# coralogix/arrow-ballista

Hardware: AMD Instinct MI355X
Metric: tpch_sf100_q3_lineitem_rows_per_sec (higher is better)
Workload: dtype i128; 1 GPU; TPC-H SF100 q3 (BASELINE configs[2]): filter x3 + hash join customer|x|orders + hash join |x| lineitem + aggregate + sort, one task on 1 x MI355X; lineitem_rows=600037902, lineitem_rows_per_gpu=600037902, orders_rows_per_gpu=150009476, customer_rows_per_gpu=15000000, input=Arrow-physical columns resident in HBM, parallelism=single partition

## Files before the change

### arrow-ballista_amd/csrc/capi.cpp

```cpp
#include "../../include/gpuq.h"
#include "expr_compile.h"
#include "agg_compile.h"
#include "gpuq_kernels.h"
#include "jit_runtime.h"
#include "devbuf.h"
#include "gpuq_internal.h"
#include <hip/hip_runtime.h>
#include <algorithm>
#include <memory>
#include <mutex>
#include <cctype>
#include <cstdio>
#include <cstdlib>
#include <cstring>
#include <string>
#include <tuple>
#include <map>
#include <deque>
#include <functional>
#include <vector>

using namespace gpuq;

namespace {
// ... 15 lines not shown
  Schema in_schema;
  CompiledProgram prog;
  DevBuf code_dev, flags_dev;
  std::vector<gpuq_field_info> out_fields;
  std::string mode = "Single", strategy = "auto";
  AggSpec agg{}; KeySpec keys{};
  std::vector<DType> key_types, acc_types;
  std::vector<int> acc_bits;
  std::map<std::pair<const void*, int>, int> jit_runs;
  std::map<std::tuple<const void*, int, size_t>, const JitFn*> jit_fns;
  struct PostChunk { CompiledProgram prog; DevBuf code; int first_out = 0; };
  std::deque<PostChunk> posts; Schema post_schema;
  i64 expected_groups = 0;
  int join_type = JT_INNER; int null_eq = 0; bool build_side_rows = true;
  bool has_semi = false; KeySpec semi_keys{};
  SortSpec sort{}; i64 fetch = -1;
  uint32_t nparts = 0;
  struct { void* data = nullptr; u64* valid = nullptr; bool done = false; } sort_dec;
  DType sort_key0;
  std::string refuse;
  std::string label;
  bool deferred = false, defer_client = false;
  struct Learned {
    struct { bool valid = false, dense = false, sparse_bits = false, has_dups = false; i64 kmin = 0; u64 krange = 0; } jb;
    struct { bool valid = false; int path = 0, gmax = 0; u64 est = 0; bool use_lds = false; i64 groups = -1; } ag;
    struct { bool valid = false; SortPack K{}; int total = 0; } so;
    bool join_guess_failed = false, sort_guess_failed = false;
    uint32_t expect_flags = 0;
    void forget() { jb.valid = ag.valid = so.valid = false; }
  } learned;
  DevBuf ws[10];
  uint32_t* pin = nullptr;
  uint32_t* pinned() { if (!pin) { if (hipHostMalloc((void**)&pin, 256, hipHostMallocDefault) != hipSuccess) { (void)hipGetLastError(); pin = nullptr; } } return pin; }
  bool profile = false; hipEvent_t ev0 = nullptr, ev1 = nullptr; float kernel_ms = 0; int launches = 0; bool ev_pending = false;
  hipEvent_t ev2 = nullptr, ev3 = nullptr; float total_ms = 0, last_total_ms = 0; bool ev_total_pending = false;
  ~gpuq_op() { for (hipEvent_t e : {ev0, ev1, ev2, ev3}) if (e) (void)hipEventDestroy(e); if (pin) (void)hipHostFree(pin); }
};

struct gpuq_join_table {
  gpuq_ctx* ctx = nullptr;
  KeySpec keys{}; HashTable T{}; int null_eq = 0; bool has_present = true;
  DevBuf slots, dense, dense_bits, next, visited, present, ws_bitmap, ws_counts;
  i64 bound = 0;
  bool visited_ready = false;
  bool has_dups = false;
};

// ... 48 lines not shown
  return P;
}

void need_exact_rows(const gpuq_input* in, const char* what) {
  if (in && in->n_rows_dev) throw std::runtime_error(std::string(what) + ": the input carries a device-side row count (n_rows_dev); this entry point needs the exact count");
}
void reset_flags(gpuq_op* op, hipStream_t s) { HIPCHECK(hipMemsetAsync(op->flags_dev.p, 0, 4, s)); }
void read_status(gpuq_op* op, hipStream_t s, uint32_t* out, int n) {
  uint32_t* h = op->pinned();
  HIPCHECK(hipMemcpyAsync(h ? h : out, op->flags_dev.p, (size_t)n * 4, hipMemcpyDeviceToHost, s));
  HIPCHECK(hipStreamSynchronize(s));
  if (h) for (int i = 0; i < n; ++i) out[i] = h[i];
}
uint32_t read_flags(gpuq_op* op, hipStream_t s) { uint32_t f = 0; read_status(op, s, &f, 1); return f; }
void raise_flags(uint32_t f) {
  if (f & FLAG_STR_TRUNC) throw Unsupported("a Utf8 value longer than 15 bytes reached a device string comparison/key (PACKED15 limit)");
  if (f & FLAG_DEC_OVERFLOW) throw std::runtime_error("decimal arithmetic overflow: a result or a rescaled operand does not fit Decimal128 (38 digits / 127 bits)");
  if (f & FLAG_WIDE_MINMAX) throw Unsupported("MIN/MAX over a value outside the int64 range is not supported on device");
  if (f & FLAG_DUP_BUILD_KEY) throw Unsupported("duplicate build keys without a chain buffer");
  if (f & FLAG_OUT_OVERFLOW) throw Capacity("join output capacity exceeded; see the pair count for the required size");
  if (f & FLAG_TABLE_FULL) throw std::runtime_error("hash table full");
  if (f & FLAG_GROUP_OVERFLOW) throw Capacity("group capacity exceeded");
  if (f & FLAG_SORT_LAYOUT) throw std::runtime_error("a row does not fit the remembered sort key layout");
}

struct ProfScope {
  gpuq_op* op; hipStream_t s;
  ProfScope(gpuq_op* o, hipStream_t st) : op(o), s(st) {
    if (op->profile) {
      if (!op->ev0) { HIPCHECK(hipEventCreate(&op->ev0)); HIPCHECK(hipEventCreate(&op->ev1)); }
      if (op->ev_pending) { float ms = 0; HIPCHECK(hipEventSynchronize(op->ev1)); HIPCHECK(hipEventElapsedTime(&ms, op->ev0, op->ev1)); op->kernel_ms += ms; op->ev_pending = false; }
      HIPCHECK(hipEventRecord(op->ev0, s));
    }
  }
  ~ProfScope() { if (op->profile) { (void)hipEventRecord(op->ev1, s); op->ev_pending = true; op->launches++; } }
};

struct ProfTotal {
  gpuq_op* op; hipStream_t s; bool on = false;
  ProfTotal(gpuq_op* o, hipStream_t st) : op(o), s(st) {
    if (op->profile) {
      if (!op->ev2) { HIPCHECK(hipEventCreate(&op->ev2)); HIPCHECK(hipEventCreate(&op->ev3)); }
      if (op->ev_total_pending) {
        if (hipEventQuery(op->ev3) != hipSuccess) { (void)hipGetLastError(); return; }
        float ms = 0; HIPCHECK(hipEventElapsedTime(&ms, op->ev2, op->ev3)); op->total_ms += ms; op->ev_total_pending = false;
      }
// ... 739 lines not shown
          cnt = std::min<u64>(cnt * (u64)wstep, (u64)n);
        }
        const u64 lim = std::max<u64>((u64)cnt * (u64)dense_ratio, 1ull << 16);
        if (span < (1ull << 31) && span < lim && (span + 1) * 4 <= op->ctx->hbm / 8) { dense = true; kmin = lo; krange = span + 1; sparse_bits = cnt * 4 < krange; }
      }
    }
    t->T.dense = nullptr; t->T.dense_bits = nullptr; t->T.dense_min = 0; t->T.dense_range = 0;
    if (dense) {
      t->T.n_slots = 0; t->T.slots = nullptr;
      t->T.dense = (uint32_t*)t->dense.ensure((size_t)krange * 4 + 16); t->T.dense_min = kmin; t->T.dense_range = krange;
      if (sparse_bits) {
        const size_t bb = ((size_t)krange + 63) / 64 * 8 + 8;
        t->T.dense_bits = (uint32_t*)t->dense_bits.ensure(bb);
        HIPCHECK(hipMemsetAsync(t->T.dense_bits, 0, bb, s));
      } else HIPCHECK(hipMemsetAsync(t->T.dense, 0xFF, (size_t)krange * 4, s));
    } else {
      t->T.n_slots = next_pow2(std::max<u64>((u64)n * 3, 1024));
      t->T.slots = (u64*)t->slots.ensure((size_t)t->T.n_slots * t->T.slot_words * 8);
    }
    uint32_t* next = (!memo || jb.has_dups) ? (uint32_t*)t->next.ensure((size_t)std::max<i64>(build_rows_bound, 1) * 4) : nullptr;
    const size_t bm = ((size_t)build_rows_bound + 63) / 64 * 8 + 8;
    uint32_t* present = op->build_side_rows ? (uint32_t*)t->present.ensure(bm) : nullptr;
    t->has_present = op->build_side_rows;
    auto build = [&]() {
      if (present) HIPCHECK(hipMemsetAsync(present, 0, bm, s));
      if (!dense) launch_ht_init(s, t->T, nullptr);
      if (!memo) reset_flags(op, s);
      if (rows_out) HIPCHECK(hipMemsetAsync(rows_out, 0, 8, s));
      { SinkJit jit(op, op->prog, GPUQ_SINK_JOIN_BUILD, n, semi_spec(t->T, present)); ProfScope ps(op, s); if (!launch_join_build(s, jit.fn, P, n, op->keys, t->T, next, present, payload_via, op->null_eq, semi_p)) throw Unsupported("join build over a semi table: more than 8 input columns without the specialised kernel"); }
      HIPCHECK(hipGetLastError());
    };
    build();
    if (memo) { t->has_dups = jb.has_dups; return true; }
    uint32_t f = read_flags(op, s);
    if (guess && (f & FLAG_TABLE_FULL)) { reset_flags(op, s); return false; }
    if (sparse_bits && (f & FLAG_DUP_BUILD_KEY)) {
      t->T.dense_bits = nullptr;
      HIPCHECK(hipMemsetAsync(t->T.dense, 0xFF, (size_t)krange * 4, s));
      build();
      f = read_flags(op, s);
    }
    if (f & ~FLAG_DUP_BUILD_KEY) { reset_flags(op, s); raise_flags(f & ~FLAG_DUP_BUILD_KEY); }
    if (f) reset_flags(op, s);
    t->has_dups = (f & FLAG_DUP_BUILD_KEY) != 0;
    jb = {true, dense, t->T.dense_bits != nullptr, t->has_dups, kmin, krange};
    op->learned.expect_flags = t->has_dups ? FLAG_DUP_BUILD_KEY : 0u;
    return true;
    };
    bool built = false;
    static const bool trace = getenv("GPUQ_TRACE_JOIN_BUILD") != nullptr;
    if (op->deferred && op->learned.jb.valid) { built = attempt(2); if (trace) fprintf(stderr, "[gpuq] join build: %lld rows (bound), deferred with the remembered layout\n", (long long)n); }
    else if (in->n_rows_dev) throw std::runtime_error("join build: a device-side row count needs a deferred operator with a completed synchronous run (gpuq_op_can_defer)");
    if (!built && spec_on && narrow_key && n >= (1ll << 21) && !op->learned.join_guess_failed) { built = attempt(true); if (!built) op->learned.join_guess_failed = true; if (trace) fprintf(stderr, "[gpuq] join build: %lld rows, guessed range %s\n", (long long)n, built ? "held" : "did not hold"); }
    if (!built) { attempt(false); if (trace) fprintf(stderr, "[gpuq] join build: %lld rows, measured range, %s\n", (long long)n, t->T.dense ? (t->T.dense_bits ? "array + bitmap" : "array") : "hash table"); }
    *out = t;
  });
  if (rc != GPUQ_OK) { delete t; if (out) *out = nullptr; }
  return rc;
}
int gpuq_join_build_run(gpuq_op* op, void* stream, const gpuq_input* in, int payload_via, int64_t build_rows_bound, gpuq_join_table** out) {
  return join_build_impl(op, stream, in, payload_via, build_rows_bound, nullptr, nullptr, nullptr, out);
}
int gpuq_join_build_run_semi(gpuq_op* op, void* stream, const gpuq_input* in, int payload_via, int64_t build_rows_bound, gpuq_join_table* semi_table,
                             uint32_t* semi_hits_out, uint64_t* rows_out, gpuq_join_table** out) {
  if (!semi_table) return GPUQ_ERR_INVALID;
  return join_build_impl(op, stream, in, payload_via, build_rows_bound, semi_table, semi_hits_out, rows_out, out);
}
int gpuq_join_table_has_duplicates(const gpuq_join_table* t) { return t && t->has_dups ? 1 : 0; }
// ... 900 lines not shown
```

### arrow-ballista_amd/csrc/gpuq_dev.h

```cpp
#pragma once
#ifndef __HIPCC_RTC__
#include <hip/hip_runtime.h>
#include <stdint.h>
#else
typedef signed char int8_t;
typedef unsigned char uint8_t;
typedef signed short int16_t;
typedef unsigned short uint16_t;
typedef signed int int32_t;
typedef unsigned int uint32_t;
#endif

namespace gpuq {

typedef unsigned long long u64;
typedef long long i64;
typedef __int128 i128;
typedef unsigned __int128 u128;

constexpr int MAX_COLS = 16;
constexpr int NREG = 16;
constexpr int MAX_INSNS = 192;
constexpr int MAX_IMMS = 48;
constexpr int MAX_VIA = 3;
// ... 59 lines not shown
  const uint32_t* via[MAX_VIA];
  const DevCode* code;
  uint32_t* flags;
  const u64* n_dev;
};
#ifdef GPUQ_NT_STREAM
#define GPUQ_LD_STREAM(p) __builtin_nontemporal_load(p)
#else
#define GPUQ_LD_STREAM(p) (*(p))
#endif
__device__ __forceinline__ i64 rows_of(const DevProgram& P, const i64 n_bound) {
  if (P.n_dev) { const i64 nd = (i64)*P.n_dev; return nd < n_bound ? nd : n_bound; }
  return n_bound;
}

constexpr uint32_t FLAG_STR_TRUNC = 1u;
constexpr uint32_t FLAG_GROUP_OVERFLOW = 2u;
constexpr uint32_t FLAG_TABLE_FULL = 4u;
constexpr uint32_t FLAG_DUP_BUILD_KEY = 8u;
constexpr uint32_t FLAG_OUT_OVERFLOW = 16u;
constexpr uint32_t FLAG_WIDE_MINMAX = 32u;
constexpr uint32_t FLAG_DEC_OVERFLOW = 128u;
constexpr uint32_t FLAG_SORT_LAYOUT = 64u;

#define GPUQ_REGS_DECL ::gpuq::u64 rlo[::gpuq::NREG]; ::gpuq::u64 rhi[::gpuq::NREG]; uint32_t rnulls = 0
#define GPUQ_REGS_PARAM ::gpuq::u64 (&rlo)[::gpuq::NREG], ::gpuq::u64 (&rhi)[::gpuq::NREG], uint32_t& rnulls
#define GPUQ_REGS_CPARAM const ::gpuq::u64 (&rlo)[::gpuq::NREG], const ::gpuq::u64 (&rhi)[::gpuq::NREG], const uint32_t& rnulls
#define GPUQ_REGS rlo, rhi, rnulls

__device__ __forceinline__ i128 mk128(u64 lo, u64 hi) { return (i128)(((u128)hi << 64) | (u128)lo); }

__device__ __forceinline__ i64 f64_total_key(u64 bits) {
  i64 s = (i64)bits;
  return s ^ (i64)((u64)(s >> 63) >> 1);
}

__device__ __forceinline__ void str15_assemble(u64 w0, u64 w1, u64 w2, uint32_t byte_off, int32_t n, u64& hi, u64& lo) {
  hi = 0; lo = 0;
  if (n <= 0) return;
  const uint32_t sh = byte_off * 8u;
  u64 s0 = sh ? ((w0 >> sh) | (w1 << (64u - sh))) : w0;
  u64 s1 = sh ? ((w1 >> sh) | (w2 << (64u - sh))) : w1;
  if (n < 8) { s0 &= (1ull << (8 * n)) - 1; s1 = 0; }
  else if (n == 8) s1 = 0;
  else s1 &= (1ull << (8 * (n - 8))) - 1;
  hi = __builtin_bswap64(s0); lo = __builtin_bswap64(s1);
// ... 323 lines not shown
```

### arrow-ballista_amd/csrc/gpuq_kernels.h

```cpp
#pragma once
#include "gpuq_dev.h"
#ifndef GPUQ_JIT
#include <type_traits>
#include "devbuf.h"
#endif

namespace gpuq {

constexpr int MAX_OUTS = 16;
struct OutCol {
  void* data;
  u64* validity;
  int32_t reg;
  int32_t cls;
};
struct OutSpec { int32_t n_out; int32_t pad; OutCol cols[MAX_OUTS]; };

constexpr int MAX_ACCS = 12;
constexpr int MAX_KEYS = 4;
enum AccKind : int32_t { ACC_SUM = 0, ACC_COUNT = 1, ACC_COUNT_STAR = 2, ACC_MIN = 3, ACC_MAX = 4, ACC_FSUM = 5, ACC_FMIN = 6, ACC_FMAX = 7 };
struct AggSpec {
  int32_t n_keys, n_accs;
  int32_t key_reg[MAX_KEYS];
  int32_t acc_kind[MAX_ACCS];
// ... 6 lines not shown



constexpr int MAX_KW = 2 * MAX_KEYS + 1;
struct KeySpec {
  int32_t n_keys;
  int32_t key_reg[MAX_KEYS];
  int32_t key_wide[MAX_KEYS];
  int32_t null_word;
  int32_t key_words;
  int32_t word_reg[MAX_KW];
  int32_t word_half[MAX_KW];
};
struct HashTable {
  u64* slots;
  u64 n_slots;
  int32_t slot_words;
  int32_t key_words;
  uint32_t* dense;
  i64 dense_min;
  u64 dense_range;
  uint32_t* dense_bits;
};
struct SemiProbe { HashTable T; KeySpec K; int32_t null_eq; int32_t on; uint32_t* hit_out; u64* rows_out; };
enum JoinType : int32_t { JT_INNER = 0, JT_LEFT = 1, JT_RIGHT = 2, JT_FULL = 3, JT_LEFT_SEMI = 4, JT_LEFT_ANTI = 5, JT_RIGHT_SEMI = 6, JT_RIGHT_ANTI = 7 };


constexpr uint32_t NIL = 0xFFFFFFFFu;
__device__ __forceinline__ uint32_t tag_of(u64 h) { return (uint32_t)(h >> 32) | 2u; }

__device__ __forceinline__ u64 acc_identity(const int kind, const int half) {
  switch (kind) {
    case ACC_MIN: return half ? 0 : 0x7FFFFFFFFFFFFFFFull;
    case ACC_MAX: return half ? ~0ull : 0x8000000000000000ull;
    case ACC_FMIN: return half ? 0 : 0x7FF0000000000000ull;
    case ACC_FMAX: return half ? 0 : 0xFFF0000000000000ull;
    default: return 0;
  }
}
__device__ __forceinline__ u64 slot_word_identity(const AggSpec& A, const int w, const int cell0) {
  const int a = (w - cell0) >> 1;
  return (w >= cell0 && a < A.n_accs) ? acc_identity(A.acc_kind[a], (w - cell0) & 1) : 0;
}
__device__ __forceinline__ void lds_table_init(u64* slots, const uint32_t cap, const int slot_words, const int cell0, const AggSpec& A, const uint32_t nthreads) {
  for (uint32_t i = threadIdx.x; i < cap * (uint32_t)slot_words; i += nthreads) slots[i] = slot_word_identity(A, (int)(i % (uint32_t)slot_words), cell0);
}
__device__ __forceinline__ bool acc_operand(const AggSpec& A, const int a, GPUQ_REGS_CPARAM, u64& vlo, u64& vhi) {
// ... 174 lines not shown
int agg_tiny_max_groups(int n_accs);
size_t agg_tiny_workspace_bytes(int gmax, int n_keys, int n_accs, int* nblocks_out);
void launch_agg_tiny(hipStream_t s, void* jit_fn, const DevProgram& P, i64 n, const AggSpec& A, int gmax, void* workspace);
void launch_agg_tiny_merge(hipStream_t s, const DevProgram& P, i64 n, const AggSpec& A, int gmax, void* workspace, const AggOut& out);
void launch_ht_init(hipStream_t s, const HashTable& T, const AggSpec* A);
void launch_agg_hash(hipStream_t s, void* jit_fn, const DevProgram& P, i64 n, const KeySpec& K, const AggSpec& A, const HashTable& T);
void launch_key_sample(hipStream_t s, const DevProgram& P, i64 n, const KeySpec& K, i64 stride, i64 nsample, uint32_t* bitmap, u64 nbits, unsigned long long* passed);
uint32_t agg_lds_slots(const HashTable& T);
int agg_lds_grid(i64 n);
void launch_agg_lds(hipStream_t s, void* jit_fn, const DevProgram& P, i64 n, const KeySpec& K, const AggSpec& A, const HashTable& T, u64* fstage, int n_fsum);
void launch_agg_bucket_id(hipStream_t s, void* jit_fn, const DevProgram& P, i64 n, const KeySpec& K, u64 bucket_mask, u64* bid, uint32_t* ids);
void launch_bucket_bounds(hipStream_t s, const u64* sorted_bid, i64 n, u64 nbuckets, uint32_t* bounds, int shift);
void launch_agg_bucket(hipStream_t s, void* jit_fn, const DevProgram& P, const KeySpec& K, const AggSpec& A, const uint32_t* ids, const uint32_t* bounds, uint32_t nbuckets,
                       uint32_t cap, int slot_words, const AggOut& out);
void launch_agg_hash_extract(hipStream_t s, const KeySpec& K, const AggSpec& A, const HashTable& T, const AggOut& out, uint32_t* flags);
bool launch_join_build(hipStream_t s, void* jit_fn, const DevProgram& P, i64 n, const KeySpec& K, const HashTable& T, uint32_t* next, uint32_t* present,
                       int payload_via, int null_equals_null, const SemiProbe* semi = nullptr);
void launch_join_keyrange(hipStream_t s, void* jit_fn, const DevProgram& P, i64 n, const KeySpec& K, int null_equals_null, u64* out, i64 wstep = 1);
void launch_join_probe_unique(hipStream_t s, void* jit_fn, const DevProgram& P, i64 n, const KeySpec& K, const HashTable& T, int join_type, int null_equals_null, int payload_via,
                              uint32_t* seg_build, uint32_t* seg_probe, uint32_t* seg_counts, int nsegs, i64 wpw, uint32_t* visited);
void launch_copy_segments(hipStream_t s, const uint32_t* seg_build, const uint32_t* seg_probe, const uint32_t* seg_offsets, int nsegs, i64 wpw, i64 n,
                          const u64* total, uint32_t* out_build, uint32_t* out_probe, u64 out_cap, uint32_t* flags);
void launch_join_locality(hipStream_t s, const DevProgram& P, i64 n, const KeySpec& K, const HashTable& T, i64 stride, i64 nsample, u64* out);
struct RjGeomHost { uint32_t nparts, shift; i64 tile; int32_t nblocks; };
void rj_geometry(i64 n, u64 range, int slice_log2, RjGeomHost* g);
size_t rj_hist_entries(const RjGeomHost& g);
void launch_rj_partition(hipStream_t s, void* jit_fn, const DevProgram& P, i64 n, const KeySpec& K, const HashTable& T, int payload_via, const RjGeomHost& g,
                         u64* rec, u64* rec_out, int32_t* hist, void* scan_ws, size_t scan_ws_bytes);
int rj_probe_geometry(i64 n, i64* wpw_out);
void launch_rj_probe(hipStream_t s, const u64* rec, const int32_t* n_live, const HashTable& T, int join_type, uint32_t* seg_build, uint32_t* seg_probe,
                     uint32_t* seg_counts, int nblocks, i64 wpw);
void launch_bitmap_select(hipStream_t s, const u64* present, const u64* visited, int matched, i64 nwords, i64 n, u64* bitmap,
                          uint32_t* block_counts, int nblocks, i64 wpb);
void launch_join_probe(hipStream_t s, void* jit_fn, const DevProgram& P, i64 n, const KeySpec& K, const HashTable& T, const uint32_t* next,
                       int join_type, int payload_via, int null_equals_null, uint32_t* out_build, uint32_t* out_probe,
                       u64 out_cap, u64* out_count, uint32_t* visited);
int sort_minmax_blocks(i64 n);
void launch_sort_minmax(hipStream_t s, void* jit_fn, const DevProgram& P, i64 n, const SortSpec& S, u64* out, int nblocks, i64 wstep = 1);
int sort_max_passes();
void launch_sort_pack(hipStream_t s, void* jit_fn, const DevProgram& P, i64 n, const SortSpec& S, const SortPack& K, u64* key_lo, u64* key_hi, uint32_t* ids, u64* hist, int hist_passes);
void launch_part_pid(hipStream_t s, void* jit_fn, const DevProgram& P, i64 n, const KeySpec& K, uint32_t nparts, u64* pid_out, uint32_t* ids);
void launch_part_offsets(hipStream_t s, const u64* pid, i64 n, uint32_t nparts, uint32_t* counts_ws, u64* offsets_out, int shift);
void launch_counts_to_ghist(hipStream_t s, const uint32_t* counts, uint32_t np, u64* ghist);
void launch_gather_u64(hipStream_t s, const u64* src, const uint32_t* idx, i64 n, u64* dst);
int sort_small_max();
int sort_direct_max();
// ... 110 lines not shown
```

### arrow-ballista_amd/csrc/kernels_hash.hip

```cpp
#include "gpuq_kernels.h"

namespace gpuq {

constexpr int HBLOCK = 256;
constexpr int HWAVES = HBLOCK / 64;

__device__ __forceinline__ int hlane() { return threadIdx.x & 63; }
__device__ __forceinline__ int hwave() { return threadIdx.x >> 6; }

__device__ __forceinline__ u64 a_load(const u64* p) { return __hip_atomic_load(p, __ATOMIC_RELAXED, __HIP_MEMORY_SCOPE_AGENT); }
__device__ __forceinline__ void a_store(u64* p, u64 v) { __hip_atomic_store(p, v, __ATOMIC_RELAXED, __HIP_MEMORY_SCOPE_AGENT); }
__device__ __forceinline__ u64 a_cas(u64* p, u64 expected, u64 desired) {
  __hip_atomic_compare_exchange_strong(p, &expected, desired, __ATOMIC_RELAXED, __ATOMIC_RELAXED, __HIP_MEMORY_SCOPE_AGENT);
  return expected;
}
__device__ __forceinline__ u64 a_add(u64* p, u64 v) { return __hip_atomic_fetch_add(p, v, __ATOMIC_RELAXED, __HIP_MEMORY_SCOPE_AGENT); }

__device__ __forceinline__ bool make_key(const KeySpec& K, GPUQ_REGS_CPARAM, u64 (&kw)[MAX_KW], u64& hash) {
  uint32_t knull = 0;
  u64 h = 0x243F6A8885A308D3ull;
#pragma unroll
  for (int k = 0; k < MAX_KEYS; ++k) {
    if (k < K.n_keys) {
      const int r = __builtin_amdgcn_readfirstlane(K.key_reg[k]);
// ... 514 lines not shown
  uint32_t payload;
  return ht_find(T, kw, h, payload) ? payload : NIL;
}

__device__ __forceinline__ void build_insert_dense(const DevProgram& P, const HashTable& T, uint32_t* __restrict__ next, const u64 idx, const uint32_t row) {
  bool inserted; uint32_t old = NIL;
  if (T.dense_bits) {
    const uint32_t bit = 1u << (idx & 31);
    const uint32_t was = atomicOr(T.dense_bits + (idx >> 5), bit);
    T.dense[idx] = row;
    inserted = !(was & bit);
  } else {
    old = __hip_atomic_exchange(T.dense + idx, row, __ATOMIC_RELAXED, __HIP_MEMORY_SCOPE_AGENT);
    inserted = old == NIL;
  }
  if (inserted) {
    if (next) next[row] = NIL;
  } else {
    if (!(__hip_atomic_load(P.flags, __ATOMIC_RELAXED, __HIP_MEMORY_SCOPE_AGENT) & FLAG_DUP_BUILD_KEY)) atomicOr(P.flags, FLAG_DUP_BUILD_KEY);
    if (next) next[row] = old;
  }
}
constexpr int BUILD_QCAP = 128;
template <int MAXC, bool SEMI>
__device__ __forceinline__ void k_join_build_body(const DevProgram P, const i64 n_arg, const KeySpec K, const HashTable T,
                                                       uint32_t* __restrict__ next, uint32_t* __restrict__ present, const int payload_via,
                                                       const int null_eq, const SemiProbe S) {
  const i64 n = rows_of(P, n_arg);
  __shared__ uint32_t q_pos[SEMI ? HWAVES : 1][SEMI ? BUILD_QCAP : 1], q_idx[SEMI ? HWAVES : 1][SEMI ? BUILD_QCAP : 1], q_aux[SEMI ? HWAVES : 1][SEMI ? BUILD_QCAP : 1];
  const bool queued = SEMI && S.on && T.dense != nullptr;
  const bool s_bits = S.T.dense != nullptr && S.T.dense_bits != nullptr;
  uint32_t qn = 0, survivors = 0;
  const int wv = SEMI ? hwave() : 0;
  auto flush = [&](const uint32_t from, const uint32_t cnt) {
    const bool on = (uint32_t)hlane() < cnt;
    const uint32_t j = from + (on ? (uint32_t)hlane() : 0u);
    const uint32_t pos = q_pos[wv][j], idx = q_idx[wv][j], aux = q_aux[wv][j];
    if (on) {
      if (S.hit_out) S.hit_out[pos] = s_bits ? S.T.dense[aux] : aux;
      build_insert_dense(P, T, next, (u64)idx, pos);
    }
  };
  for_rows_in_flight<MAXC>(P, n, (i64)blockIdx.x * HWAVES + hwave(), (i64)gridDim.x * HWAVES, [&](const i64 w, const i64 pos, bool active, GPUQ_REGS_PARAM) {
    uint32_t aux = NIL;
    if (SEMI && S.on) {
      bool found = false;
      if (active) {
        u64 kw1[MAX_KW]; u64 h1;
#pragma unroll
        for (int q = 0; q < MAX_KW; ++q) kw1[q] = 0;
        const bool null1 = make_key(S.K, GPUQ_REGS, kw1, h1);
        if (!(null1 && !S.null_eq)) {
          if (s_bits && queued) {
            const u64 i1 = kw1[0] - (u64)S.T.dense_min;
            if (i1 < S.T.dense_range && ((S.T.dense_bits[i1 >> 5] >> (i1 & 31)) & 1u)) { found = true; aux = (uint32_t)i1; }
          } else { aux = join_lookup(S.T, kw1, h1); found = aux != NIL; }
        }
      }
      active = active && found;
      if (!queued && active && S.hit_out) S.hit_out[pos] = aux;
      if (S.rows_out) survivors += active ? 1u : 0u;
    }
    if (present && payload_via == 0) { const u64 am = __ballot(active); if (hlane() == 0) ((u64*)present)[w] = am; }
    if (queued) {
      u64 idx = 0; bool ins = false;
      if (active) {
        u64 kw[MAX_KW]; u64 h;
#pragma unroll
        for (int q = 0; q < MAX_KW; ++q) kw[q] = 0;
        const bool any_null = make_key(K, GPUQ_REGS, kw, h);
        idx = kw[0] - (u64)T.dense_min;
        ins = !(any_null && !null_eq);
        if (ins && idx >= T.dense_range) { atomicOr(P.flags, FLAG_TABLE_FULL); ins = false; }
        if (!ins && S.hit_out) S.hit_out[pos] = s_bits ? S.T.dense[aux] : aux;
      }
      const u64 m = __ballot(ins);
      if (ins) {
        const uint32_t j = qn + (uint32_t)__popcll(m & ((1ull << hlane()) - 1));
        q_pos[wv][j] = (uint32_t)pos; q_idx[wv][j] = (uint32_t)idx; q_aux[wv][j] = aux;
      }
      qn += (uint32_t)__popcll(m);
      __builtin_amdgcn_fence(__ATOMIC_RELEASE, "wavefront"); __builtin_amdgcn_wave_barrier(); __builtin_amdgcn_fence(__ATOMIC_ACQUIRE, "wavefront");
      if (qn >= 64) { qn -= 64; flush(qn, 64); __builtin_amdgcn_wave_barrier(); }
      return;
    }
    if (!active) return;
    u64 kw[MAX_KW]; u64 h;
#pragma unroll
    for (int q = 0; q < MAX_KW; ++q) kw[q] = 0;
    const bool any_null = make_key(K, GPUQ_REGS, kw, h);
    uint32_t row = (uint32_t)pos;
    if (payload_via > 0) { row = P.via[payload_via - 1][pos]; if (present) atomicOr(&present[row >> 5], 1u << (row & 31)); }
    if (any_null && !null_eq) return;
    if (T.dense) {
      const u64 idx = kw[0] - (u64)T.dense_min;
      if (idx >= T.dense_range) { atomicOr(P.flags, FLAG_TABLE_FULL); return; }
      build_insert_dense(P, T, next, idx, row);
      return;
    }
    bool inserted; uint32_t old = NIL;
    const u64 s = ht_find_or_insert(T, kw, h, row, inserted);
    if (s == ~0ull) { atomicOr(P.flags, FLAG_TABLE_FULL); return; }
    if (!inserted && next) {
      uint32_t* head = (uint32_t*)(T.slots + s * (u64)T.slot_words) + 1;
      old = __hip_atomic_exchange(head, row, __ATOMIC_RELAXED, __HIP_MEMORY_SCOPE_AGENT);
    }
    if (inserted) {
      if (next) next[row] = NIL;
    } else {
      if (!(__hip_atomic_load(P.flags, __ATOMIC_RELAXED, __HIP_MEMORY_SCOPE_AGENT) & FLAG_DUP_BUILD_KEY)) atomicOr(P.flags, FLAG_DUP_BUILD_KEY);
      if (next) next[row] = old;
    }
  });
  if (queued && qn > 0) flush(0, qn);
  if (SEMI && S.on && S.rows_out) {
#pragma unroll
    for (int o = 32; o > 0; o >>= 1) survivors += __shfl_xor(survivors, o);
    if (hlane() == 0 && survivors) atomicAdd((unsigned long long*)S.rows_out, (unsigned long long)survivors);
  }
}
#if defined(GPUQ_JIT) && defined(GPUQ_JIT_SEMI) && GPUQ_JIT_SEMI == 2
template <int MAXC>
__device__ __forceinline__ void k_join_build_semi1_body(const DevProgram P, const i64 n_arg, const HashTable T, uint32_t* __restrict__ next, const SemiProbe S) {
#ifndef GPUQ_SEMI_ROWS
#define GPUQ_SEMI_ROWS 4
#endif
  constexpr int U = GPUQ_SEMI_ROWS;
  constexpr int QC = 64 * (U + 1);
  __shared__ uint32_t q_pos[HWAVES][QC], q_idx[HWAVES][QC], q_aux[HWAVES][QC];
  const i64 n = rows_of(P, n_arg);
  const i64 nwords = (n + 63) >> 6;
  const int wv = hwave();
  const bool s_dense = S.T.dense != nullptr;
  const uint32_t* __restrict__ sbits = S.T.dense_bits;
  const bool late_row = s_dense && sbits != nullptr;
  uint32_t qn = 0, survivors = 0;
  auto flush = [&](const uint32_t from, const uint32_t cnt) {
    const bool on = (uint32_t)hlane() < cnt;
    const uint32_t j = from + (on ? (uint32_t)hlane() : 0u);
    const uint32_t pos = q_pos[wv][j], idx = q_idx[wv][j], aux = q_aux[wv][j];
    if (on) {
      if (S.hit_out) S.hit_out[pos] = late_row ? S.T.dense[aux] : aux;
      build_insert_dense(P, T, next, (u64)idx, pos);
    }
  };
  const i64 wave0 = ((i64)blockIdx.x * HWAVES + hwave()) * U, wstride = (i64)gridDim.x * HWAVES * U;
  for (i64 wb = wave0; wb < nwords; wb += wstride) {
    bool act[U]; u64 key1[U], key2[U]; bool n1[U], n2[U]; i64 posc[U];
    {
      JitPre jq[U]; JitRaw jw[U];
#pragma unroll
      for (int u = 0; u < U; ++u) {
        const i64 pos = ((wb + u) << 6) + hlane();
        act[u] = (wb + u) < nwords && pos < n;
        posc[u] = act[u] ? pos : n - 1;
        gpuq_jit_pre(P, posc[u], jq[u]);
      }
#pragma unroll
      for (int u = 0; u < U; ++u) gpuq_jit_load(P, posc[u], jq[u], jw[u]);
#pragma unroll
      for (int u = 0; u < U; ++u) {
        GPUQ_REGS_DECL;
        const bool pass = gpuq_jit_compute(P, posc[u], jw[u], GPUQ_REGS);
        act[u] = act[u] && pass;
        n1[u] = (rnulls >> JIT_KEY_REG0) & 1; n2[u] = (rnulls >> JIT_KEY2_REG) & 1;
        key1[u] = rlo[JIT_KEY_REG0]; key2[u] = rlo[JIT_KEY2_REG];
      }
    }
    uint32_t aux[U]; bool found[U];
    if (s_dense) {
      uint32_t bw[U]; u64 i1[U]; bool in[U];
#pragma unroll
      for (int u = 0; u < U; ++u) {
        i1[u] = key1[u] - (u64)S.T.dense_min;
        in[u] = act[u] && !n1[u] && i1[u] < S.T.dense_range;
        bw[u] = 0;
        if (in[u]) bw[u] = sbits ? sbits[i1[u] >> 5] : S.T.dense[i1[u]];
      }
#pragma unroll
      for (int u = 0; u < U; ++u) {
        if (sbits) { found[u] = in[u] && ((bw[u] >> (i1[u] & 31)) & 1u); aux[u] = (uint32_t)i1[u]; }
        else { found[u] = in[u] && bw[u] != NIL; aux[u] = bw[u]; }
      }
    } else {
#pragma unroll
      for (int u = 0; u < U; ++u) {
        aux[u] = NIL;
        if (act[u] && !n1[u]) { u64 kw1[MAX_KW]; for (int q = 0; q < MAX_KW; ++q) kw1[q] = 0; kw1[0] = key1[u]; aux[u] = join_lookup(S.T, kw1, hash_combine(0x243F6A8885A308D3ull, key1[u], 0, false)); }
        found[u] = aux[u] != NIL;
      }
    }
#pragma unroll
    for (int u = 0; u < U; ++u) {
      const bool surv = act[u] && found[u];
      survivors += surv ? 1u : 0u;
      const u64 idx = key2[u] - (u64)T.dense_min;
      bool ins = surv && !n2[u];
      if (ins && idx >= T.dense_range) { atomicOr(P.flags, FLAG_TABLE_FULL); ins = false; }
      if (surv && !ins && S.hit_out) S.hit_out[posc[u]] = late_row ? S.T.dense[aux[u]] : aux[u];
      const u64 m = __ballot(ins);
      if (ins) {
        const uint32_t j = qn + (uint32_t)__popcll(m & ((1ull << hlane()) - 1));
        q_pos[wv][j] = (uint32_t)posc[u]; q_idx[wv][j] = (uint32_t)idx; q_aux[wv][j] = aux[u];
      }
      qn += (uint32_t)__popcll(m);
    }
    __builtin_amdgcn_fence(__ATOMIC_RELEASE, "wavefront"); __builtin_amdgcn_wave_barrier(); __builtin_amdgcn_fence(__ATOMIC_ACQUIRE, "wavefront");
    while (qn >= 64) { qn -= 64; flush(qn, 64); }
    __builtin_amdgcn_wave_barrier();
  }
  if (qn > 0) flush(0, qn);
  if (S.rows_out) {
#pragma unroll
    for (int o = 32; o > 0; o >>= 1) survivors += __shfl_xor(survivors, o);
    if (hlane() == 0 && survivors) atomicAdd((unsigned long long*)S.rows_out, (unsigned long long)survivors);
  }
}
#endif
#ifndef GPUQ_JIT
template <int MAXC, bool SEMI>
__global__ void __launch_bounds__(HBLOCK) k_join_build(const DevProgram P, const i64 n, const KeySpec K, const HashTable T,
                                                       uint32_t* __restrict__ next, uint32_t* __restrict__ present, const int payload_via,
                                                       const int null_eq, const SemiProbe S) { k_join_build_body<MAXC, SEMI>(P, n, K, T, next, present, payload_via, null_eq, S); }
#elif GPUQ_JIT_KERNEL == GPUQ_SINK_JOIN_BUILD
#ifndef GPUQ_JIT_SEMI
#define GPUQ_JIT_SEMI 0
#endif
extern "C" __global__ void __launch_bounds__(HBLOCK) gpuq_jit_entry(const DevProgram P, const i64 n, const KeySpec K, const HashTable T,
                                                       uint32_t* __restrict__ next, uint32_t* __restrict__ present, const int payload_via,
                                                       const int null_eq, const SemiProbe S) {
#if GPUQ_JIT_SEMI == 2
  k_join_build_semi1_body<0>(P, n, T, next, S);
#else
  k_join_build_body<0, GPUQ_JIT_SEMI != 0>(P, n, K, T, next, present, payload_via, null_eq, S);
#endif
}
#endif

template <int MAXC>
__device__ __forceinline__ void k_join_probe_body(const DevProgram P, const i64 n_arg, const KeySpec K, const HashTable T,
                                                       const uint32_t* __restrict__ next, const int join_type, const int payload_via,
                                                       const int null_eq, uint32_t* __restrict__ out_build, uint32_t* __restrict__ out_probe,
                                                       const u64 out_cap, u64* __restrict__ out_count, uint32_t* __restrict__ visited) {
  const i64 n = rows_of(P, n_arg);
  const i64 nwords = (n + 63) >> 6;
  const bool emit_pairs = (join_type == JT_INNER || join_type == JT_LEFT || join_type == JT_RIGHT || join_type == JT_FULL);
  const bool probe_outer = (join_type == JT_RIGHT || join_type == JT_FULL);
  const bool mark = (visited != nullptr);
  for (i64 w = (i64)blockIdx.x * HWAVES + hwave(); w < nwords; w += (i64)gridDim.x * HWAVES) {
    const i64 pos = (w << 6) + hlane();
    bool active = pos < n;
    GPUQ_REGS_DECL;
    if (active) active = GPUQ_EVAL(MAXC, P, pos);
    uint32_t cur = NIL;
    uint32_t prow = (uint32_t)pos;
    if (active) {
      if (payload_via > 0) prow = P.via[payload_via - 1][pos];
      u64 kw[MAX_KW]; u64 h;
// ... 518 lines not shown
}
void launch_bucket_bounds(hipStream_t s, const u64* sorted_bid, i64 n, u64 nbuckets, uint32_t* bounds, int shift) {
  const u64 need = (nbuckets + 1 + HBLOCK - 1) / HBLOCK;
  hipLaunchKernelGGL(k_bucket_bounds, dim3((unsigned)(need < 4096 ? need : 4096)), dim3(HBLOCK), 0, s, sorted_bid, n, nbuckets, bounds, shift);
}
void launch_agg_bucket(hipStream_t s, void* jit_fn, const DevProgram& P, const KeySpec& K, const AggSpec& A, const uint32_t* ids, const uint32_t* bounds, uint32_t nbuckets,
                       uint32_t cap, int slot_words, const AggOut& out) {
  const size_t lds = (size_t)cap * slot_words * 8;
  u64 grid = nbuckets; const u64 gcap = (u64)num_cus() * 8; if (grid > gcap) grid = gcap; if (grid < 1) grid = 1;
  launch_sink(jit_fn, P.n_cols, GPUQ_PICK(k_agg_bucket), dim3((unsigned)grid), dim3(HBLOCK), lds, s, P, K, A, ids, bounds, nbuckets, cap, slot_words, out);
}
bool launch_join_build(hipStream_t s, void* jit_fn, const DevProgram& P, i64 n, const KeySpec& K, const HashTable& T, uint32_t* next, uint32_t* present,
                       int payload_via, int null_equals_null, const SemiProbe* semi) {
  if (n <= 0) return true;
  SemiProbe S{}; if (semi) S = *semi;
  if (semi && !jit_fn && P.n_cols > 8) return false;
  const auto semi_pick = [](auto M) { return &k_join_build<(decltype(M)::value < 8 ? decltype(M)::value : 8), true>; };
  const auto plain_pick = [](auto M) { return &k_join_build<decltype(M)::value, false>; };
  const dim3 grid(hgrid(n, 8)), block(HBLOCK);
  if (semi) launch_sink(jit_fn, P.n_cols, semi_pick, grid, block, 0, s, P, n, K, T, next, present, payload_via, null_equals_null, S);
  else launch_sink(jit_fn, P.n_cols, plain_pick, grid, block, 0, s, P, n, K, T, next, present, payload_via, null_equals_null, S);
  return true;
}

#ifndef GPUQ_JIT
__global__ void __launch_bounds__(HBLOCK) k_bitmap_select(const u64* __restrict__ present, const u64* __restrict__ visited, const int matched,
                                                          const i64 nwords, const i64 n, u64* __restrict__ bitmap,
                                                          uint32_t* __restrict__ block_counts, const i64 wpb) {
  __shared__ uint32_t wc[HWAVES];
  const i64 w0 = (i64)blockIdx.x * wpb;
  i64 w1 = w0 + wpb; if (w1 > nwords) w1 = nwords;
  uint32_t cnt = 0;
  for (i64 w = w0 + threadIdx.x; w < w1; w += HBLOCK) {
    u64 m = present[w] & (matched ? visited[w] : ~visited[w]);
    if (w == nwords - 1 && (n & 63)) m &= (1ull << (n & 63)) - 1;
    bitmap[w] = m; cnt += (uint32_t)__popcll(m);
  }
  for (int off = 32; off > 0; off >>= 1) cnt += __shfl_xor(cnt, off);
  if (hlane() == 0) wc[hwave()] = cnt;
  __syncthreads();
  if (threadIdx.x == 0) { uint32_t t = 0; for (int k = 0; k < HWAVES; ++k) t += wc[k]; block_counts[blockIdx.x] = t; }
}
#endif
void launch_bitmap_select(hipStream_t s, const u64* present, const u64* visited, int matched, i64 nwords, i64 n, u64* bitmap,
                          uint32_t* block_counts, int nblocks, i64 wpb) {
  hipLaunchKernelGGL(k_bitmap_select, dim3(nblocks), dim3(HBLOCK), 0, s, present, visited, matched, nwords, n, bitmap, block_counts, wpb);
// ... 69 lines not shown
```

Before: 158.3 billion rows/s.

## Replace atomic OR into dense bitmap with plain stores when build keys are ordered

Adds per-wave order bookkeeping during the semi-filtered dense join build. It records the first and last key of each step, and a follow-up check kernel verifies that build keys rise strictly across the whole input. Once a build is known to be ordered, later memoized builds combine bits within a wave and write interior bitmap words with plain stores, keeping atomics only at run edges. The aim is to cut atomic traffic on the dense bitmap, at the cost of writing edge records, an extra check kernel per build, and a new failure flag if the order assumption breaks.

New measurement: 139.1 billion rows/s. 0.879x the previous value.

```diff
diff --git a/arrow-ballista_amd/csrc/capi.cpp b/arrow-ballista_amd/csrc/capi.cpp
--- a/arrow-ballista_amd/csrc/capi.cpp
+++ b/arrow-ballista_amd/csrc/capi.cpp
@@ -61,7 +61,7 @@
   std::string label;
   bool deferred = false, defer_client = false;
   struct Learned {
-    struct { bool valid = false, dense = false, sparse_bits = false, has_dups = false; i64 kmin = 0; u64 krange = 0; } jb;
+    struct { bool valid = false, dense = false, sparse_bits = false, has_dups = false; i64 kmin = 0; u64 krange = 0; bool ordered = false; } jb;
     struct { bool valid = false; int path = 0, gmax = 0; u64 est = 0; bool use_lds = false; i64 groups = -1; } ag;
     struct { bool valid = false; SortPack K{}; int total = 0; } so;
     bool join_guess_failed = false, sort_guess_failed = false;
@@ -156,6 +156,7 @@
   if (f & FLAG_TABLE_FULL) throw std::runtime_error("hash table full");
   if (f & FLAG_GROUP_OVERFLOW) throw Capacity("group capacity exceeded");
   if (f & FLAG_SORT_LAYOUT) throw std::runtime_error("a row does not fit the remembered sort key layout");
+  if (f & FLAG_BUILD_UNORDERED) throw std::runtime_error("the build keys are not in the order the remembered build relies on");
 }
 
 struct ProfScope {
@@ -941,20 +942,26 @@
     const size_t bm = ((size_t)build_rows_bound + 63) / 64 * 8 + 8;
     uint32_t* present = op->build_side_rows ? (uint32_t*)t->present.ensure(bm) : nullptr;
     t->has_present = op->build_side_rows;
+    const bool order_book = semi_p && dense && sparse_bits && payload_via == 0 && (!memo || jb.ordered);
+    semi.edges = order_book ? (BuildEdge*)op->ws[1].ensure((((size_t)n + 63) / 64 + 1) * sizeof(BuildEdge)) : nullptr;
+    semi.ordered = memo && order_book ? 1 : 0;
     auto build = [&]() {
       if (present) HIPCHECK(hipMemsetAsync(present, 0, bm, s));
       if (!dense) launch_ht_init(s, t->T, nullptr);
       if (!memo) reset_flags(op, s);
       if (rows_out) HIPCHECK(hipMemsetAsync(rows_out, 0, 8, s));
       { SinkJit jit(op, op->prog, GPUQ_SINK_JOIN_BUILD, n, semi_spec(t->T, present)); ProfScope ps(op, s); if (!launch_join_build(s, jit.fn, P, n, op->keys, t->T, next, present, payload_via, op->null_eq, semi_p)) throw Unsupported("join build over a semi table: more than 8 input columns without the specialised kernel"); }
+      if (semi.edges) launch_build_order_check(s, semi.edges, n, P.flags);
       HIPCHECK(hipGetLastError());
     };
     build();
     if (memo) { t->has_dups = jb.has_dups; return true; }
     uint32_t f = read_flags(op, s);
     if (guess && (f & FLAG_TABLE_FULL)) { reset_flags(op, s); return false; }
+    const bool ordered = order_book && !(f & (FLAG_BUILD_UNORDERED | FLAG_DUP_BUILD_KEY));
+    if (f & FLAG_BUILD_UNORDERED) { reset_flags(op, s); f &= ~FLAG_BUILD_UNORDERED; }
     if (sparse_bits && (f & FLAG_DUP_BUILD_KEY)) {
-      t->T.dense_bits = nullptr;
+      t->T.dense_bits = nullptr; semi.edges = nullptr;
       HIPCHECK(hipMemsetAsync(t->T.dense, 0xFF, (size_t)krange * 4, s));
       build();
       f = read_flags(op, s);
@@ -962,7 +969,7 @@
     if (f & ~FLAG_DUP_BUILD_KEY) { reset_flags(op, s); raise_flags(f & ~FLAG_DUP_BUILD_KEY); }
     if (f) reset_flags(op, s);
     t->has_dups = (f & FLAG_DUP_BUILD_KEY) != 0;
-    jb = {true, dense, t->T.dense_bits != nullptr, t->has_dups, kmin, krange};
+    jb = {true, dense, t->T.dense_bits != nullptr, t->has_dups, kmin, krange, ordered};
     op->learned.expect_flags = t->has_dups ? FLAG_DUP_BUILD_KEY : 0u;
     return true;
     };
diff --git a/arrow-ballista_amd/csrc/gpuq_dev.h b/arrow-ballista_amd/csrc/gpuq_dev.h
--- a/arrow-ballista_amd/csrc/gpuq_dev.h
+++ b/arrow-ballista_amd/csrc/gpuq_dev.h
@@ -105,6 +105,7 @@
 constexpr uint32_t FLAG_WIDE_MINMAX = 32u;
 constexpr uint32_t FLAG_DEC_OVERFLOW = 128u;
 constexpr uint32_t FLAG_SORT_LAYOUT = 64u;
+constexpr uint32_t FLAG_BUILD_UNORDERED = 256u;
 
 #define GPUQ_REGS_DECL ::gpuq::u64 rlo[::gpuq::NREG]; ::gpuq::u64 rhi[::gpuq::NREG]; uint32_t rnulls = 0
 #define GPUQ_REGS_PARAM ::gpuq::u64 (&rlo)[::gpuq::NREG], ::gpuq::u64 (&rhi)[::gpuq::NREG], uint32_t& rnulls
diff --git a/arrow-ballista_amd/csrc/gpuq_kernels.h b/arrow-ballista_amd/csrc/gpuq_kernels.h
--- a/arrow-ballista_amd/csrc/gpuq_kernels.h
+++ b/arrow-ballista_amd/csrc/gpuq_kernels.h
@@ -52,7 +52,8 @@
   u64 dense_range;
   uint32_t* dense_bits;
 };
-struct SemiProbe { HashTable T; KeySpec K; int32_t null_eq; int32_t on; uint32_t* hit_out; u64* rows_out; };
+struct alignas(16) BuildEdge { uint32_t first, last, any, pad; };
+struct SemiProbe { HashTable T; KeySpec K; int32_t null_eq; int32_t on; uint32_t* hit_out; u64* rows_out; BuildEdge* edges; int32_t ordered; };
 enum JoinType : int32_t { JT_INNER = 0, JT_LEFT = 1, JT_RIGHT = 2, JT_FULL = 3, JT_LEFT_SEMI = 4, JT_LEFT_ANTI = 5, JT_RIGHT_SEMI = 6, JT_RIGHT_ANTI = 7 };
 
 
@@ -273,6 +274,7 @@
 void launch_copy_segments(hipStream_t s, const uint32_t* seg_build, const uint32_t* seg_probe, const uint32_t* seg_offsets, int nsegs, i64 wpw, i64 n,
                           const u64* total, uint32_t* out_build, uint32_t* out_probe, u64 out_cap, uint32_t* flags);
 void launch_join_locality(hipStream_t s, const DevProgram& P, i64 n, const KeySpec& K, const HashTable& T, i64 stride, i64 nsample, u64* out);
+void launch_build_order_check(hipStream_t s, const BuildEdge* edges, i64 n_bound, uint32_t* flags);
 struct RjGeomHost { uint32_t nparts, shift; i64 tile; int32_t nblocks; };
 void rj_geometry(i64 n, u64 range, int slice_log2, RjGeomHost* g);
 size_t rj_hist_entries(const RjGeomHost& g);
diff --git a/arrow-ballista_amd/csrc/kernels_hash.hip b/arrow-ballista_amd/csrc/kernels_hash.hip
--- a/arrow-ballista_amd/csrc/kernels_hash.hip
+++ b/arrow-ballista_amd/csrc/kernels_hash.hip
@@ -560,6 +560,64 @@
   }
 }
 constexpr int BUILD_QCAP = 128;
+constexpr uint32_t BUILD_Q_INTERIOR = 0x80000000u;
+template <int QC> struct BuildQueue { uint32_t* pos; uint32_t* idx; uint32_t* aux; uint32_t head, tail; };
+template <int QC>
+__device__ __forceinline__ void build_queue_push(BuildQueue<QC>& q, const bool ins, const uint32_t pos, const uint32_t entry, const uint32_t aux) {
+  const u64 m = __ballot(ins);
+  if (ins) {
+    const uint32_t j = (q.tail + (uint32_t)__popcll(m & ((1ull << hlane()) - 1))) % (uint32_t)QC;
+    q.pos[j] = pos; q.idx[j] = entry; q.aux[j] = aux;
+  }
+  q.tail += (uint32_t)__popcll(m);
+}
+template <int QC>
+__device__ __forceinline__ void build_queue_flush(BuildQueue<QC>& q, const uint32_t cnt, const bool ordered, const DevProgram& P, const HashTable& T,
+                                                  uint32_t* __restrict__ next, const SemiProbe& S, const bool late_row) {
+  const int lane = hlane();
+  const bool on = (uint32_t)lane < cnt;
+  const uint32_t j = (q.head + (on ? (uint32_t)lane : 0u)) % (uint32_t)QC;
+  const uint32_t pos = q.pos[j], entry = q.idx[j], aux = q.aux[j];
+  q.head += cnt;
+  const uint32_t idx = entry & ~BUILD_Q_INTERIOR;
+  if (on && S.hit_out) S.hit_out[pos] = late_row ? S.T.dense[aux] : aux;
+  if (!ordered) { if (on) build_insert_dense(P, T, next, (u64)idx, pos); return; }
+  const uint32_t word = on ? idx >> 5 : 0xFFFFFFFFu;
+  uint32_t bits = on ? 1u << (idx & 31) : 0u;
+  bool interior = (entry & BUILD_Q_INTERIOR) != 0;
+  const uint32_t pw = __shfl_up(word, 1), nw = __shfl_down(word, 1);
+  const bool head = lane == 0 || pw != word, tail = lane == 63 || nw != word;
+  bool f = head;
+#pragma unroll
+  for (int off = 1; off < 64; off <<= 1) {
+    const uint32_t ub = __shfl_up(bits, off);
+    const bool ui = __shfl_up((int)interior, off) != 0, uf = __shfl_up((int)f, off) != 0;
+    if (lane >= off && !f) { bits |= ub; interior = interior && ui; f = uf; }
+  }
+  const u64 tails = __ballot(on && tail);
+  if (on) {
+    T.dense[idx] = pos;
+    if (next) next[pos] = NIL;
+    if (tail) {
+      const bool edge_run = lane == __builtin_ctzll(tails) || (uint32_t)lane == cnt - 1;
+      if (interior && !edge_run) T.dense_bits[word] = bits;
+      else (void)__hip_atomic_fetch_or(T.dense_bits + word, bits, __ATOMIC_RELAXED, __HIP_MEMORY_SCOPE_AGENT);
+    }
+  }
+}
+struct StepOrder { uint32_t first, last; bool any; };
+__device__ __forceinline__ bool step_order_word(StepOrder& o, const bool p, const uint32_t k) {
+  const u64 m = __ballot(p);
+  if (m == 0) return false;
+  const u64 below = m & ((1ull << hlane()) - 1);
+  const uint32_t pk = (uint32_t)__shfl((int)k, below ? 63 - __builtin_clzll(below) : 0);
+  const bool bad = p && (below ? pk >= k : (o.any && o.last >= k));
+  if (!o.any) o.first = (uint32_t)__builtin_amdgcn_readlane((int)k, __builtin_ctzll(m));
+  o.last = (uint32_t)__builtin_amdgcn_readlane((int)k, 63 - __builtin_clzll(m));
+  o.any = true;
+  return bad;
+}
+__device__ __forceinline__ bool step_interior(const StepOrder& o, const uint32_t idx) { return (idx >> 5) > (o.first >> 5) && (idx >> 5) < (o.last >> 5); }
 template <int MAXC, bool SEMI>
 __device__ __forceinline__ void k_join_build_body(const DevProgram P, const i64 n_arg, const KeySpec K, const HashTable T,
                                                        uint32_t* __restrict__ next, uint32_t* __restrict__ present, const int payload_via,
@@ -568,19 +626,16 @@
   __shared__ uint32_t q_pos[SEMI ? HWAVES : 1][SEMI ? BUILD_QCAP : 1], q_idx[SEMI ? HWAVES : 1][SEMI ? BUILD_QCAP : 1], q_aux[SEMI ? HWAVES : 1][SEMI ? BUILD_QCAP : 1];
   const bool queued = SEMI && S.on && T.dense != nullptr;
   const bool s_bits = S.T.dense != nullptr && S.T.dense_bits != nullptr;
-  uint32_t qn = 0, survivors = 0;
+  uint32_t survivors = 0;
   const int wv = SEMI ? hwave() : 0;
-  auto flush = [&](const uint32_t from, const uint32_t cnt) {
-    const bool on = (uint32_t)hlane() < cnt;
-    const uint32_t j = from + (on ? (uint32_t)hlane() : 0u);
-    const uint32_t pos = q_pos[wv][j], idx = q_idx[wv][j], aux = q_aux[wv][j];
-    if (on) {
-      if (S.hit_out) S.hit_out[pos] = s_bits ? S.T.dense[aux] : aux;
-      build_insert_dense(P, T, next, (u64)idx, pos);
-    }
-  };
+  BuildQueue<BUILD_QCAP> Q{q_pos[wv], q_idx[wv], q_aux[wv], 0u, 0u};
+  const bool book = queued && S.edges != nullptr;
+  const bool ordered = book && S.ordered != 0;
+  bool unordered = false;
+  if (book && blockIdx.x == 0 && threadIdx.x == 0) S.edges[0] = BuildEdge{(uint32_t)((n + 63) >> 6), 0u, 0u, 0u};
   for_rows_in_flight<MAXC>(P, n, (i64)blockIdx.x * HWAVES + hwave(), (i64)gridDim.x * HWAVES, [&](const i64 w, const i64 pos, bool active, GPUQ_REGS_PARAM) {
     uint32_t aux = NIL;
+    bool passing = false;
     if (SEMI && S.on) {
       bool found = false;
       if (active) {
@@ -595,31 +650,36 @@
           } else { aux = join_lookup(S.T, kw1, h1); found = aux != NIL; }
         }
       }
+      passing = active;
       active = active && found;
       if (!queued && active && S.hit_out) S.hit_out[pos] = aux;
       if (S.rows_out) survivors += active ? 1u : 0u;
     }
     if (present && payload_via == 0) { const u64 am = __ballot(active); if (hlane() == 0) ((u64*)present)[w] = am; }
     if (queued) {
-      u64 idx = 0; bool ins = false;
+      u64 idx = 0; bool ins = false, any_null = false;
+      if (active || (book && passing)) {
+        u64 kw[MAX_KW]; u64 h;
+#pragma unroll
+        for (int q = 0; q < MAX_KW; ++q) kw[q] = 0;
+        any_null = make_key(K, GPUQ_REGS, kw, h);
+        idx = kw[0] - (u64)T.dense_min;
+      }
       if (active) {
-        u64 kw[MAX_KW]; u64 h;
-#pragma unroll
-        for (int q = 0; q < MAX_KW; ++q) kw[q] = 0;
-        const bool any_null = make_key(K, GPUQ_REGS, kw, h);
-        idx = kw[0] - (u64)T.dense_min;
         ins = !(any_null && !null_eq);
         if (ins && idx >= T.dense_range) { atomicOr(P.flags, FLAG_TABLE_FULL); ins = false; }
         if (!ins && S.hit_out) S.hit_out[pos] = s_bits ? S.T.dense[aux] : aux;
       }
-      const u64 m = __ballot(ins);
-      if (ins) {
-        const uint32_t j = qn + (uint32_t)__popcll(m & ((1ull << hlane()) - 1));
-        q_pos[wv][j] = (uint32_t)pos; q_idx[wv][j] = (uint32_t)idx; q_aux[wv][j] = aux;
-      }
-      qn += (uint32_t)__popcll(m);
+      StepOrder so{0u, 0u, false};
+      if (book) {
+        unordered = unordered || (passing && (any_null || idx >= T.dense_range));
+        const bool bad = step_order_word(so, passing, (uint32_t)idx);
+        unordered = unordered || bad;
+        if (hlane() == 0) S.edges[1 + w] = BuildEdge{so.first, so.last, so.any ? 1u : 0u, 0u};
+      }
+      build_queue_push(Q, ins, (uint32_t)pos, (uint32_t)idx | (book && step_interior(so, (uint32_t)idx) ? BUILD_Q_INTERIOR : 0u), aux);
       __builtin_amdgcn_fence(__ATOMIC_RELEASE, "wavefront"); __builtin_amdgcn_wave_barrier(); __builtin_amdgcn_fence(__ATOMIC_ACQUIRE, "wavefront");
-      if (qn >= 64) { qn -= 64; flush(qn, 64); __builtin_amdgcn_wave_barrier(); }
+      if (Q.tail - Q.head >= 64u) { build_queue_flush(Q, 64u, ordered, P, T, next, S, s_bits); __builtin_amdgcn_wave_barrier(); }
       return;
     }
     if (!active) return;
@@ -650,7 +710,8 @@
       if (next) next[row] = old;
     }
   });
-  if (queued && qn > 0) flush(0, qn);
+  if (queued && Q.tail != Q.head) build_queue_flush(Q, Q.tail - Q.head, ordered, P, T, next, S, s_bits);
+  if (book && __ballot(unordered) != 0 && hlane() == 0) atomicOr(P.flags, FLAG_BUILD_UNORDERED);
   if (SEMI && S.on && S.rows_out) {
 #pragma unroll
     for (int o = 32; o > 0; o >>= 1) survivors += __shfl_xor(survivors, o);
@@ -672,16 +733,12 @@
   const bool s_dense = S.T.dense != nullptr;
   const uint32_t* __restrict__ sbits = S.T.dense_bits;
   const bool late_row = s_dense && sbits != nullptr;
-  uint32_t qn = 0, survivors = 0;
-  auto flush = [&](const uint32_t from, const uint32_t cnt) {
-    const bool on = (uint32_t)hlane() < cnt;
-    const uint32_t j = from + (on ? (uint32_t)hlane() : 0u);
-    const uint32_t pos = q_pos[wv][j], idx = q_idx[wv][j], aux = q_aux[wv][j];
-    if (on) {
-      if (S.hit_out) S.hit_out[pos] = late_row ? S.T.dense[aux] : aux;
-      build_insert_dense(P, T, next, (u64)idx, pos);
-    }
-  };
+  uint32_t survivors = 0;
+  BuildQueue<QC> Q{q_pos[wv], q_idx[wv], q_aux[wv], 0u, 0u};
+  const bool book = S.edges != nullptr;
+  const bool ordered = book && S.ordered != 0;
+  bool unordered = false;
+  if (book && blockIdx.x == 0 && threadIdx.x == 0) S.edges[0] = BuildEdge{(uint32_t)((nwords + U - 1) / U), 0u, 0u, 0u};
   const i64 wave0 = ((i64)blockIdx.x * HWAVES + hwave()) * U, wstride = (i64)gridDim.x * HWAVES * U;
   for (i64 wb = wave0; wb < nwords; wb += wstride) {
     bool act[U]; u64 key1[U], key2[U]; bool n1[U], n2[U]; i64 posc[U];
@@ -727,6 +784,17 @@
         if (act[u] && !n1[u]) { u64 kw1[MAX_KW]; for (int q = 0; q < MAX_KW; ++q) kw1[q] = 0; kw1[0] = key1[u]; aux[u] = join_lookup(S.T, kw1, hash_combine(0x243F6A8885A308D3ull, key1[u], 0, false)); }
         found[u] = aux[u] != NIL;
       }
+    }
+    StepOrder so{0u, 0u, false};
+    if (book) {
+#pragma unroll
+      for (int u = 0; u < U; ++u) {
+        const u64 idx = key2[u] - (u64)T.dense_min;
+        unordered = unordered || (act[u] && (n2[u] || idx >= T.dense_range));
+        const bool bad = step_order_word(so, act[u], (uint32_t)idx);
+        unordered = unordered || bad;
+      }
+      if (hlane() == 0) S.edges[1 + wb / U] = BuildEdge{so.first, so.last, so.any ? 1u : 0u, 0u};
     }
 #pragma unroll
     for (int u = 0; u < U; ++u) {
@@ -736,18 +804,14 @@
       bool ins = surv && !n2[u];
       if (ins && idx >= T.dense_range) { atomicOr(P.flags, FLAG_TABLE_FULL); ins = false; }
       if (surv && !ins && S.hit_out) S.hit_out[posc[u]] = late_row ? S.T.dense[aux[u]] : aux[u];
-      const u64 m = __ballot(ins);
-      if (ins) {
-        const uint32_t j = qn + (uint32_t)__popcll(m & ((1ull << hlane()) - 1));
-        q_pos[wv][j] = (uint32_t)posc[u]; q_idx[wv][j] = (uint32_t)idx; q_aux[wv][j] = aux[u];
-      }
-      qn += (uint32_t)__popcll(m);
+      build_queue_push(Q, ins, (uint32_t)posc[u], (uint32_t)idx | (book && step_interior(so, (uint32_t)idx) ? BUILD_Q_INTERIOR : 0u), aux[u]);
     }
     __builtin_amdgcn_fence(__ATOMIC_RELEASE, "wavefront"); __builtin_amdgcn_wave_barrier(); __builtin_amdgcn_fence(__ATOMIC_ACQUIRE, "wavefront");
-    while (qn >= 64) { qn -= 64; flush(qn, 64); }
+    while (Q.tail - Q.head >= 64u) build_queue_flush(Q, 64u, ordered, P, T, next, S, late_row);
     __builtin_amdgcn_wave_barrier();
   }
-  if (qn > 0) flush(0, qn);
+  if (Q.tail != Q.head) build_queue_flush(Q, Q.tail - Q.head, ordered, P, T, next, S, late_row);
+  if (book && __ballot(unordered) != 0 && hlane() == 0) atomicOr(P.flags, FLAG_BUILD_UNORDERED);
   if (S.rows_out) {
 #pragma unroll
     for (int o = 32; o > 0; o >>= 1) survivors += __shfl_xor(survivors, o);
@@ -772,6 +836,35 @@
 #else
   k_join_build_body<0, GPUQ_JIT_SEMI != 0>(P, n, K, T, next, present, payload_via, null_eq, S);
 #endif
+}
+#endif
+
+#ifndef GPUQ_JIT
+__global__ void __launch_bounds__(HBLOCK) k_build_order_check(const BuildEdge* __restrict__ edges, uint32_t* __restrict__ flags) {
+  const i64 nsteps = (i64)edges[0].first;
+  const uint4* __restrict__ e = (const uint4*)(edges + 1);
+  const int lane = hlane();
+  bool bad = false;
+  for (i64 base = ((i64)blockIdx.x * HWAVES + hwave()) << 6; base < nsteps; base += ((i64)gridDim.x * HWAVES) << 6) {
+    const i64 i = base + lane;
+    uint4 me = make_uint4(0u, 0u, 0u, 0u);
+    if (i < nsteps) me = e[i];
+    const bool any = me.z != 0;
+    const u64 m = __ballot(any);
+    if (m == 0) continue;
+    const u64 below = m & ((1ull << lane) - 1);
+    uint32_t prev = (uint32_t)__shfl((int)me.y, below ? 63 - __builtin_clzll(below) : 0);
+    bool has_prev = below != 0;
+    uint32_t carry = 0; bool have = false;
+    for (i64 b = base - 64; b >= 0 && !have; b -= 64) {
+      const uint4 o = e[b + lane];
+      const u64 mm = __ballot(o.z != 0);
+      if (mm) { carry = (uint32_t)__builtin_amdgcn_readlane((int)o.y, 63 - __builtin_clzll(mm)); have = true; }
+    }
+    if (!has_prev) { prev = carry; has_prev = have; }
+    bad = bad || (any && (me.x > me.y || (has_prev && prev >= me.x)));
+  }
+  if (__ballot(bad) != 0 && lane == 0) atomicOr(flags, FLAG_BUILD_UNORDERED);
 }
 #endif
 
@@ -1336,6 +1429,12 @@
   else launch_sink(jit_fn, P.n_cols, plain_pick, grid, block, 0, s, P, n, K, T, next, present, payload_via, null_equals_null, S);
   return true;
 }
+void launch_build_order_check(hipStream_t s, const BuildEdge* edges, i64 n_bound, uint32_t* flags) {
+  if (n_bound <= 0) return;
+  const u64 need = (((u64)n_bound + 63) / 64 + 64 * HWAVES - 1) / (64 * HWAVES);
+  const u64 cap = (u64)num_cus() * 8;
+  hipLaunchKernelGGL(k_build_order_check, dim3((unsigned)(need < cap ? need : cap)), dim3(HBLOCK), 0, s, edges, flags);
+}
 
 #ifndef GPUQ_JIT
 __global__ void __launch_bounds__(HBLOCK) k_bitmap_select(const u64* __restrict__ present, const u64* __restrict__ visited, const int matched,
```
